# ZhenghaoFei/visual_odom

Hardware: AMD Instinct MI355X
Metric: stereo frames/sec on KITTI-00 1241x376 @ ~2000 features (higher is better)
Workload: dtype u8/int32 LK (f32 2x2 solve), f64 pose solve

## Files before the change

visual_odom_amd/csrc/lk.hip:

```cpp
#include "vo_kernels.h"
#include "vo_lkmath.h"

#include <float.h>
#include <type_traits>

namespace vo {

constexpr int LK_WIN = 21;
constexpr int LK_JT_W = 48, LK_JT_H = 40;
constexpr int LK_W_BITS = 14;
template <int W>
struct LkWin {
    static_assert(W % 2 == 1 && W >= 5 && W <= LK_WIN, "odd windows of 5 .. 21: the pyramid's borders are laid out for 21");
    static constexpr int SEGS = (W + 6) / 7, LANES = W * SEGS, COLS = 7 * SEGS + 1, ROWS = W + 1, LAST = W - 7 * (SEGS - 1);
    static constexpr int OFF_X = ((LK_JT_W - COLS) / 2) & ~3, OFF_Y = (LK_JT_H - ROWS) / 2;
    static_assert(LANES <= 64 && LK_JT_W >= COLS + OFF_X + 3 && LK_JT_H >= ROWS + OFF_Y, "the lane map and the tile hold the window");
};
constexpr uint32_t lk_seg_mask(int valid, int m)
{
    return (2 * m < valid ? 0x0000ffffu : 0u) | (2 * m + 1 < valid ? 0xffff0000u : 0u);
}

__device__ __forceinline__ void lk_weights(float a, float b, uint32_t &wt, uint32_t &wb)
{
    const float s = (float)(1 << LK_W_BITS), magic = 12582912.f;
    const float a1 = (1.f - a) * s, a0 = a * s, b1 = 1.f - b;
    const uint32_t r00 = (uint32_t)__float_as_int(a1 * b1 + magic);
    const uint32_t r01 = (uint32_t)__float_as_int(a0 * b1 + magic);
    const uint32_t r10 = (uint32_t)__float_as_int(a1 * b + magic);
    const uint32_t iw11 = ((1u << LK_W_BITS) + 3u * 0x4B400000u) - (r00 + r01 + r10);
    wt = perm_b32(r01, r00, VO_SEL_LO16);
    wb = perm_b32(iw11, r10, VO_SEL_LO16);
}

struct LkOrigin {
    int x, y;
};
template <int W = LK_WIN>
__device__ __forceinline__ bool lk_tile_misses(bool have_tile, int jx0, int jy0, int inx, int iny)
{
    return !have_tile || inx < jx0 || inx + LkWin<W>::COLS > jx0 + LK_JT_W || iny < jy0 || iny + LkWin<W>::ROWS > jy0 + LK_JT_H;
}
template <int W = LK_WIN>
__device__ __forceinline__ LkOrigin lk_tile_refill(uint8_t *tile, const VO_GLOBAL uint8_t *__restrict__ Jimg, int jstride, int jx_max, int jy_max,
                                               int inx, int iny, int c0, int step)
{
    int jx0 = (inx - LkWin<W>::OFF_X) & ~3;
    int jy0 = iny - LkWin<W>::OFF_Y;
    jx0 = jx0 < -VO_BX ? -VO_BX : jx0 > jx_max ? jx_max : jx0;
    jy0 = jy0 < -VO_BY ? -VO_BY : jy0 > jy_max ? jy_max : jy0;
    const VO_GLOBAL uint8_t *tb = Jimg + (ptrdiff_t)jy0 * jstride + jx0;
    for (int c = c0; c < LK_JT_H * (LK_JT_W / 16); c += step) {
        const int row = c / (LK_JT_W / 16), col = c - row * (LK_JT_W / 16);
        const U32x4A4 v = *(const VO_GLOBAL U32x4A4 *)(tb + (uint32_t)(row * jstride + 16 * col));
        *reinterpret_cast<uint4 *>(&tile[row * LK_JT_W + 16 * col]) = make_uint4(v.a, v.b, v.c, v.d);
    }
    return LkOrigin{jx0, jy0};
}
template <int W = LK_WIN>
__device__ __forceinline__ LkOrigin lk_tile_cover(uint8_t *tile, const VO_GLOBAL uint8_t *__restrict__ Jimg, int jstride, int jx_max, int jy_max,
                                              int inx, int iny, int lane, bool have_tile, int jx0, int jy0)
{
    if (!lk_tile_misses<W>(have_tile, jx0, jy0, inx, iny))
        return LkOrigin{jx0, jy0};
    __syncthreads();
    const LkOrigin o = lk_tile_refill<W>(tile, Jimg, jstride, jx_max, jy_max, inx, iny, lane, 64);
    __syncthreads();
    return o;
}
__device__ __forceinline__ void lk_cell_rows(const uint8_t *tile, int off, uint32_t Jt[7], uint32_t Jb[7])
{
    const U32x2A1 t = *reinterpret_cast<const U32x2A1 *>(&tile[off]);
    const U32x2A1 u = *reinterpret_cast<const U32x2A1 *>(&tile[off + LK_JT_W]);
    lift7(t.a, t.b, Jt);
    lift7(u.a, u.b, Jb);
}

#ifndef VO_LK_ATTRS
#define VO_LK_ATTRS __launch_bounds__(64, 7)
#endif
constexpr int VO_LK_USE_INITIAL_FLOW = 4, VO_LK_GET_MIN_EIGENVALS = 8;
template <bool SPLIT, bool ERR, int WIN = LK_WIN, bool FLAGS = false>
__device__ __forceinline__ void lk_circular_body(const PyrImage *__restrict__ imgs, const Quad *__restrict__ quads,
                                                 const float2 *__restrict__ pts_in, const int *__restrict__ n_pts, int cap,
                                                 int n_frames, int fpg , int ppp ,
                                                 float2 *__restrict__ trk,
                                                 uint8_t *__restrict__ status,
                                                 const LkParams prm, int hop_begin, int hop_end, float *__restrict__ err = nullptr,
                                                 int flags = 0)
{
    __shared__ __attribute__((aligned(16))) uint8_t s_jt[LK_JT_H * LK_JT_W];

    const int bid = blockIdx.x;
    const int xcd = bid & 7, slot = bid >> 3;
    const int grp = slot / ppp, fi = slot - grp * ppp;
    const int frame = grp * fpg + (xcd & (fpg - 1));
    const int f = (xcd / fpg) * ppp + fi;
    if (frame >= n_frames || f >= n_pts[frame])
        return;
    const int lane = threadIdx.x;
    using LW = LkWin<WIN>;
    const bool live = lane < LW::LANES;
    const int lr = live ? lane : LW::LANES - 1;
    const int r = lr / LW::SEGS, c0 = 7 * (lr - LW::SEGS * r);
    const int lane_off = r * LK_JT_W + c0;

    const Quad q = quads[frame];
    const float halfWin = (WIN - 1) * 0.5f;
    const float FLT_SCALE = 1.f / (1 << 20);
    const float eps_lo = (float)(prm.epsilon * 0.999999), eps_hi = (float)(prm.epsilon * 1.000001);
    const float min_eig_n = prm.min_eig * (1.001f * (float)(2 * WIN * WIN));

    const float2 p = pts_in[(size_t)frame * cap + f];
    float prevPtX = unif(p.x), prevPtY = unif(p.y);
    if (SPLIT && hop_begin > 0) {
        const size_t o = ((size_t)frame * 4 + (hop_begin - 1)) * cap + f;
        const float2 q0 = trk[o];
        const bool dead0 = status[o] == 0 || q0.x < 0.f || q0.y < 0.f || (hop_begin == 1 && (p.x < 0.f || p.y < 0.f));
        if (dead0 && !prm.full_chain)
            return;
        prevPtX = unif(q0.x);
        prevPtY = unif(q0.y);
    }

    for (int hop = SPLIT ? hop_begin : 0; hop < (ERR ? 1 : SPLIT ? hop_end : 4); hop++) {
        const int pi = hop == 0 ? q.l0 : hop == 1 ? q.r0 : hop == 2 ? q.r1 : q.l1;
        const int ni = hop == 0 ? q.r0 : hop == 1 ? q.r1 : hop == 2 ? q.l1 : q.l0;
        const PyrImage &I = imgs[pi];
        const PyrImage &J = imgs[ni];
        float outX = 0.f, outY = 0.f;
        int st = 1;
        float errv = 0.f;

        for (int level = prm.max_level; level >= 0; level--) {
            const float scale = __int_as_float((127 - level) << 23);
            float prevX = prevPtX * scale, prevY = prevPtY * scale;
            float nextX, nextY;
            if (level == prm.max_level) {
                nextX = prevX;
                nextY = prevY;
                if constexpr (FLAGS) {
                    if (flags & VO_LK_USE_INITIAL_FLOW) {
                        const float2 g = trk[(size_t)frame * cap + f];
                        nextX = unif(g.x) * scale;
                        nextY = unif(g.y) * scale;
                    }
                }
            } else {
                nextX = outX * 2.f;
                nextY = outY * 2.f;
            }
            outX = nextX;
            outY = nextY;

            const int iw = I.w[level], ih = I.h[level], istride = I.stride[level];
            const int jw = J.w[level], jh = J.h[level], jstride = J.stride[level];
            const VO_GLOBAL uint8_t *__restrict__ Iimg = (const VO_GLOBAL uint8_t *)I.lvl[level];
            const VO_GLOBAL uint32_t *__restrict__ Ider = (const VO_GLOBAL uint32_t *)I.der[level];
            const VO_GLOBAL uint8_t *__restrict__ Jimg = (const VO_GLOBAL uint8_t *)J.lvl[level];

            prevX -= halfWin;
            prevY -= halfWin;
            const float fpx = floorf(prevX), fpy = floorf(prevY);
            const int ipx = uni(vo_f2i(fpx)), ipy = uni(vo_f2i(fpy));
            if (VO_BALLOT(__builtin_isunordered(fpx, fpy)) != 0ull || ipx < -WIN || ipx >= iw || ipy < -WIN || ipy >= ih) {
                if (level == 0)
                    st = 0;
                continue;
            }
            uint32_t wt, wb;
            lk_weights(prevX - fpx, prevY - fpy, wt, wb);

            uint32_t Ixp[4], Iyp[4];
            uint32_t Ipe[ERR ? 4 : 1];
            int a11 = 0, a12 = 0, a22 = 0, c1 = 0, c2 = 0;
            {
                const ptrdiff_t org = (ptrdiff_t)VO_BY * istride + VO_BX;
                const VO_GLOBAL uint8_t *Ib = Iimg - org;
                const VO_GLOBAL uint8_t *Db = (const VO_GLOBAL uint8_t *)(Ider - org);
                const uint32_t o = (uint32_t)((ipy + r + VO_BY) * istride + ipx + c0 + VO_BX);
                const uint32_t od = live ? 4u * o : 0u, drow = 4u * (uint32_t)istride;
                const U32x2A1 t = *(const VO_GLOBAL U32x2A1 *)(Ib + o);
                const U32x2A1 u = *(const VO_GLOBAL U32x2A1 *)(Ib + (o + (uint32_t)istride));
                const U32x4A4 dt0 = *(const VO_GLOBAL U32x4A4 *)(Db + od);
                const U32x4A4 dt1 = *(const VO_GLOBAL U32x4A4 *)(Db + (od + 16u));
                const U32x4A4 db0 = *(const VO_GLOBAL U32x4A4 *)(Db + (od + drow));
                const U32x4A4 db1 = *(const VO_GLOBAL U32x4A4 *)(Db + (od + drow + 16u));
                const uint32_t dt[8] = {dt0.a, dt0.b, dt0.c, dt0.d, dt1.a, dt1.b, dt1.c, dt1.d};
                const uint32_t db[8] = {db0.a, db0.b, db0.c, db0.d, db1.a, db1.b, db1.c, db1.d};
                uint32_t Ip[4];
                bilinear7_u8(t.a, t.b, u.a, u.b, wt, wb, Ip);
                bilinear7_deriv(dt, db, wt, wb, Ixp, Iyp);
                if constexpr (LW::LAST < 7) {
                    const bool part = LW::SEGS == 1 || c0 == 7 * (LW::SEGS - 1);
#pragma unroll
                    for (int m = 0; m < 4; m++) {
                        const uint32_t keep = part ? lk_seg_mask(LW::LAST, m) : 0xffffffffu;
                        Ixp[m] &= keep;
                        Iyp[m] &= keep;
                    }
                }
                a11 = sdot2_first(Ixp[0], Ixp[0], 0);
                a12 = sdot2_first(Ixp[0], Iyp[0], 0);
                a22 = sdot2_first(Iyp[0], Iyp[0], 0);
                c1 = sdot2_first(Ip[0], Ixp[0], 0);
                c2 = sdot2_first(Ip[0], Iyp[0], 0);
#pragma unroll
                for (int m = 1; m < 4; m++) {
                    a11 = sdot2(Ixp[m], Ixp[m], a11);
                    a12 = sdot2(Ixp[m], Iyp[m], a12);
                    a22 = sdot2(Iyp[m], Iyp[m], a22);
                    c1 = sdot2(Ip[m], Ixp[m], c1);
                    c2 = sdot2(Ip[m], Iyp[m], c2);
                }
                if constexpr (ERR) {
#pragma unroll
                    for (int m = 0; m < 4; m++)
                        Ipe[m] = Ip[m];
                }
            }
            float A11, A12, A22;
            wave_sum3_exact_f32(a11, a12, a22, A11, A12, A22);
            A11 *= FLT_SCALE;
            A12 *= FLT_SCALE;
            A22 *= FLT_SCALE;

            float D = A11 * A22 - A12 * A12;
            const float t = A22 + A11;
            const float s2 = (A11 - A22) * (A11 - A22) + 4.f * A12 * A12;
            const float u = t - (min_eig_n + t * 3.814697265625e-6f);
            bool eig_ok = u > 0.f && s2 < u * u * 0.9999f;
            if (__builtin_expect(!eig_ok, 0)) {
#ifndef VO_HOST_EMUL
                asm volatile("" ::: "memory");
#endif
                const float minEig = (t - sqrtf(s2)) / (float)(2 * WIN * WIN);
                eig_ok = !(minEig < prm.min_eig);
            }
            if constexpr (FLAGS) {
                if ((flags & VO_LK_GET_MIN_EIGENVALS) && level == 0)
                    errv = (t - sqrtf(s2)) / (float)(2 * WIN * WIN);
            }
            if (!eig_ok || D < FLT_EPSILON) {
                if (level == 0)
                    st = 0;
                continue;
            }
            D = 1.f / D;
            const float A11s = A11 * FLT_SCALE, A12s = A12 * FLT_SCALE, A22s = A22 * FLT_SCALE;
            const int nc1 = -c1, nc2 = -c2;

            nextX -= halfWin;
            nextY -= halfWin;
            float prevDX = 0.f, prevDY = 0.f;
            int jx0 = 0, jy0 = 0;
            bool have_tile = false;
            static_assert(LK_JT_W % 16 == 0 && VO_BX % 4 == 0, "16-byte tile chunks at 4-byte aligned origins");
            static_assert(VO_BY >= WIN && LK_JT_W >= LW::COLS + LW::OFF_X + 3 && LK_JT_H >= LW::ROWS + LW::OFF_Y,
                          "a tile clamped to the row end / the last border row still covers what the window of every corner the "
                          "reference admits reads (up to w - 1, h - 1: the borders are at least a window wide)");
            static_assert(VO_BY >= LW::COLS - 1, "right border (at least VO_BY columns) >= the columns a row reads beyond corner w - 1");
            const int jx_max = jstride - VO_BX - LK_JT_W, jy_max = jh + VO_BY - LK_JT_H;

            int j = 0;
            float fnx = floorf(nextX), fny = floorf(nextY);
            bool run = prm.max_count > 0;
            while (run) {
                const int inx = uni(vo_f2i(fnx)), iny = uni(vo_f2i(fny));
                if (VO_BALLOT(__builtin_isunordered(fnx, fny)) != 0ull || inx < -WIN || inx >= jw || iny < -WIN || iny >= jh) {
                    if (level == 0)
                        st = 0;
                    break;
                }
                {
                    const LkOrigin o = lk_tile_cover<WIN>(s_jt, Jimg, jstride, jx_max, jy_max, inx, iny, lane, have_tile, jx0, jy0);
                    jx0 = o.x;
                    jy0 = o.y;
                    have_tile = true;
                }
                uint32_t Jt[7], Jb[7];
                lk_cell_rows(s_jt, (iny - jy0) * LK_JT_W + (inx - jx0) + lane_off, Jt, Jb);
                for (;;) {
                    lk_weights(nextX - fnx, nextY - fny, wt, wb);
                    int b1, b2;
                    {
                        uint32_t Jp[4];
                        blend7(Jt, Jb, wt, wb, Jp);
                        b1 = sdot2_first(Jp[0], Ixp[0], nc1);
                        b2 = sdot2_first(Jp[0], Iyp[0], nc2);
#pragma unroll
                        for (int m = 1; m < 4; m++) {
                            b1 = sdot2(Jp[m], Ixp[m], b1);
                            b2 = sdot2(Jp[m], Iyp[m], b2);
                        }
                    }
                    float fb1, fb2;
                    wave_sum2_exact_f32(b1, b2, fb1, fb2);
                    const float dx = (A12s * fb2 - A22s * fb1) * D;
                    const float dy = (A12s * fb1 - A11s * fb2) * D;
                    nextX += dx;
                    nextY += dy;
                    outX = nextX + halfWin;
                    outY = nextY + halfWin;
                    const float n2 = fmaf(dy, dy, dx * dx);
                    if (__builtin_expect(!(n2 > eps_hi), 0)) {
#ifndef VO_HOST_EMUL
                        asm volatile("" ::: "memory");
#endif
                        if (n2 < eps_lo || (double)dx * dx + (double)dy * dy <= prm.epsilon) {
                            run = false;
                            break;
                        }
                    }
                    if (j > 0 && fabsf(dx + prevDX) <= 0.01f && fabsf(dy + prevDY) <= 0.01f) {
#ifndef VO_HOST_EMUL
                        asm volatile("" ::: "memory");
#endif
                        outX -= dx * 0.5f;
                        outY -= dy * 0.5f;
                        run = false;
                        break;
                    }
                    prevDX = dx;
                    prevDY = dy;
                    if (++j >= prm.max_count) {
                        run = false;
                        break;
                    }
                    const uint32_t ua = (uint32_t)__float_as_int(nextX - fnx), ub = (uint32_t)__float_as_int(nextY - fny);
                    if (VO_BALLOT((ua > ub ? ua : ub) >= 0x3f800000u) != 0ull) {
                        fnx = floorf(nextX);
                        fny = floorf(nextY);
                        break;
                    }
                }
            }

            if (st && level == 0 && (!FLAGS || !(flags & VO_LK_GET_MIN_EIGENVALS))) {
                const int fx = vo_f2i(floorf(outX - halfWin)), fy = vo_f2i(floorf(outY - halfWin));
                if (fx < -WIN || fx >= jw || fy < -WIN || fy >= jh)
                    st = 0;
                if constexpr (ERR) {
                    if (st && err != nullptr) {
                        const float ex = outX - halfWin, ey = outY - halfWin;
                        const float fex = floorf(ex), fey = floorf(ey);
                        const int inx = uni(fx), iny = uni(fy);
                        const LkOrigin o = lk_tile_cover<WIN>(s_jt, Jimg, jstride, jx_max, jy_max, inx, iny, lane, have_tile, jx0, jy0);
                        jx0 = o.x;
                        jy0 = o.y;
                        uint32_t Jt[7], Jb[7], Jp[4];
                        lk_cell_rows(s_jt, (iny - jy0) * LK_JT_W + (inx - jx0) + lane_off, Jt, Jb);
                        lk_weights(ex - fex, ey - fey, wt, wb);
                        blend7(Jt, Jb, wt, wb, Jp);
                        uint32_t e = 0;
#pragma unroll
                        for (int m = 0; m < 4; m++) {
                            if constexpr (LW::LAST < 7) {
                                const bool part = LW::SEGS == 1 || c0 == 7 * (LW::SEGS - 1);
                                e = udot2(pk_absdiff_i16(Jp[m], Ipe[m]) & (part ? lk_seg_mask(LW::LAST, m) : 0xffffffffu), 0x00010001u, e);
                            } else
                                e = udot2(pk_absdiff_i16(Jp[m], Ipe[m]), 0x00010001u, e);
                        }
                        errv = wave_sum_exact_f32(live ? (int)e : 0) / (float)(32 * WIN * WIN);
                    }
                }
            }
        }

        if constexpr (ERR) {
            if (lane == 0) {
                trk[(size_t)frame * cap + f] = make_float2(outX, outY);
                status[(size_t)frame * cap + f] = (uint8_t)st;
                if (err != nullptr) {
                    if constexpr (FLAGS)
                        err[(size_t)frame * cap + f] = ((flags & VO_LK_GET_MIN_EIGENVALS) || st) ? errv : 0.f;
                    else
                        err[(size_t)frame * cap + f] = st ? errv : 0.f;
                }
            }
            return;
        }
        if (lane == 0) {
            trk[((size_t)frame * 4 + hop) * cap + f] = make_float2(outX, outY);
            status[((size_t)frame * 4 + hop) * cap + f] = (uint8_t)st;
        }
        const bool dead = st == 0 || outX < 0.f || outY < 0.f || (hop == 0 && (p.x < 0.f || p.y < 0.f));
        if (dead && !prm.full_chain && hop < 3) {
            if (lane == 0)
                for (int k = hop + 1; k < 4; k++) {
                    trk[((size_t)frame * 4 + k) * cap + f] = make_float2(-1.f, -1.f);
                    status[((size_t)frame * 4 + k) * cap + f] = 0;
                }
            return;
        }
        prevPtX = unif(outX);
        prevPtY = unif(outY);
    }
}

__global__ VO_LK_ATTRS void lk_circular_kernel(const PyrImage *__restrict__ imgs,
                                                          const Quad *__restrict__ quads,
                                                          const float2 *__restrict__ pts_in,
                                                          const int *__restrict__ n_pts, int cap,
                                                          int n_frames, int fpg ,
                                                          int ppp ,
                                                          float2 *__restrict__ trk,
                                                          uint8_t *__restrict__ status,
                                                          LkParams prm)
{
    lk_circular_body<false, false>(imgs, quads, pts_in, n_pts, cap, n_frames, fpg, ppp, trk, status, prm, 0, 4);
}

__global__ VO_LK_ATTRS void lk_hops_kernel(const PyrImage *__restrict__ imgs, const Quad *__restrict__ quads,
                                           const float2 *__restrict__ pts_in, const int *__restrict__ n_pts, int cap,
                                           int n_frames, int fpg, int ppp, float2 *__restrict__ trk,
                                           uint8_t *__restrict__ status, LkParams prm, int hop_begin, int hop_end)
{
    lk_circular_body<true, false>(imgs, quads, pts_in, n_pts, cap, n_frames, fpg, ppp, trk, status, prm, hop_begin, hop_end);
}

#ifndef VO_LK_FLOW_ATTRS
#define VO_LK_FLOW_ATTRS __launch_bounds__(64, 6)
#endif
__global__ VO_LK_FLOW_ATTRS void lk_flow_kernel(const PyrImage *__restrict__ imgs, const Quad *__restrict__ pairs,
                                                const float2 *__restrict__ pts_in, const int *__restrict__ n_pts, int cap,
                                                int n_frames, int fpg, int ppp, float2 *__restrict__ next,
                                                uint8_t *__restrict__ status,
                                                float *__restrict__ err , LkParams prm)
{
    lk_circular_body<false, true>(imgs, pairs, pts_in, n_pts, cap, n_frames, fpg, ppp, next, status, prm, 0, 1, err);
}

template <int W>
__global__ VO_LK_FLOW_ATTRS void lk_flow_win_kernel(const PyrImage *__restrict__ imgs, const Quad *__restrict__ pairs,
                                                    const float2 *__restrict__ pts_in, const int *__restrict__ n_pts, int cap,
                                                    int n_frames, int fpg, int ppp, float2 *__restrict__ next,
                                                    uint8_t *__restrict__ status,
                                                    float *__restrict__ err , LkParams prm)
{
    static_assert(W < LK_WIN, "21 is lk_flow_kernel");
    lk_circular_body<false, true, W>(imgs, pairs, pts_in, n_pts, cap, n_frames, fpg, ppp, next, status, prm, 0, 1, err);
}

template <int W>
__global__ VO_LK_FLOW_ATTRS void lk_flow_flags_kernel(const PyrImage *__restrict__ imgs, const Quad *__restrict__ pairs,
                                                      const float2 *__restrict__ pts_in, const int *__restrict__ n_pts, int cap,
                                                      int n_frames, int fpg, int ppp, float2 *__restrict__ next,
                                                      uint8_t *__restrict__ status,
                                                      float *__restrict__ err , LkParams prm, int flags)
{
    lk_circular_body<false, true, W, true>(imgs, pairs, pts_in, n_pts, cap, n_frames, fpg, ppp, next, status, prm, 0, 1, err, flags);
}

struct LkGrid {
    int fpg, ppp, blocks;
};
inline LkGrid lk_grid(int n_frames, int n_items)
{
    const int fpg = n_frames >= 8 ? 8 : n_frames >= 4 ? 4 : n_frames >= 2 ? 2 : 1;
    const int parts = 8 / fpg, ppp = (n_items + parts - 1) / parts;
    const int groups = (n_frames + fpg - 1) / fpg;
    return {fpg, ppp, 8 * groups * ppp};
}

template <int... W, typename F>
inline bool lk_visit_window(int win, F &&f)
{
    return ((win == W && (f(std::integral_constant<int, W>{}), true)) || ...);
}
template <typename F>
inline bool lk_for_window(int win, F &&f)
{
    return lk_visit_window<5, 7, 9, 11, 13, 15, 17, 19, LK_WIN>(win, f);
}

template <int W, typename R>
inline void lk_flow_route(int flags, R &&run)
{
    if (flags != 0)
        run(lk_flow_flags_kernel<W>, flags);
    else if constexpr (W == LK_WIN)
        run(lk_flow_kernel);
    else
        run(lk_flow_win_kernel<W>);
}

#ifndef VO_HOST_EMUL
void launch_lk_flow(int win, int flags, const PyrImage *d_imgs, const Quad *d_pairs, const float2 *d_pts, const int *d_npts, int cap,
                    int max_pts, int n_frames, float2 *d_next, uint8_t *d_status, float *d_err, const LkParams &prm, hipStream_t stream)
{
    if (max_pts <= 0 || n_frames <= 0 || (flags & ~(VO_LK_USE_INITIAL_FLOW | VO_LK_GET_MIN_EIGENVALS)))
        return;
    const LkGrid g = lk_grid(n_frames, max_pts);
    lk_for_window(win, [&](auto w) {
        lk_flow_route<decltype(w)::value>(flags, [&](auto kernel, auto... tail) {
            hipLaunchKernelGGL(kernel, dim3((unsigned)g.blocks), dim3(64), 0, stream, d_imgs, d_pairs, d_pts, d_npts, cap, n_frames, g.fpg,
                               g.ppp, d_next, d_status, d_err, prm, tail...);
        });
    });
}

void launch_lk_circular(const PyrImage *d_imgs, const Quad *d_quads, const float2 *d_pts, const int *d_npts,
                        int cap, int max_pts, int n_frames, float2 *d_trk, uint8_t *d_status,
                        const LkParams &prm, hipStream_t stream)
{
    if (max_pts <= 0 || n_frames <= 0)
        return;
    const LkGrid g = lk_grid(n_frames, max_pts);
    hipLaunchKernelGGL(lk_circular_kernel, dim3((unsigned)g.blocks), dim3(64), 0, stream, d_imgs, d_quads, d_pts, d_npts, cap,
                       n_frames, g.fpg, g.ppp, d_trk, d_status, prm);
}

void launch_lk_hops(const PyrImage *d_imgs, const Quad *d_quads, const float2 *d_pts, const int *d_npts, int cap, int max_pts,
                    int n_frames, float2 *d_trk, uint8_t *d_status, const LkParams &prm, int hop_begin, int hop_end,
                    hipStream_t stream)
{
    if (max_pts <= 0 || n_frames <= 0 || hop_begin < 0 || hop_end > 4 || hop_begin >= hop_end)
        return;
    const LkGrid g = lk_grid(n_frames, max_pts);
    hipLaunchKernelGGL(lk_hops_kernel, dim3((unsigned)g.blocks), dim3(64), 0, stream, d_imgs, d_quads, d_pts, d_npts, cap, n_frames,
                       g.fpg, g.ppp, d_trk, d_status, prm, hop_begin, hop_end);
}

#endif

}

#ifdef VO_HOST_EMUL
#include "dev/lk_dev.hip"
#endif
```

visual_odom_amd/csrc/vo_lkmath.h:

```cpp
#pragma once

#include "vo_isa.h"

namespace vo {

#define VO_SEL_PIX(k) (0x0cu | ((uint32_t)(k) << 8) | (0x0cu << 16) | ((uint32_t)((k) + 1) << 24))
constexpr uint32_t VO_SEL_LO16 = 0x05040100u;
constexpr uint32_t VO_SEL_HI16 = 0x07060302u;

VO_HD uint32_t pack_w(int w_lo, int w_hi)
{
#if defined(__HIP_DEVICE_COMPILE__)
    return __builtin_bit_cast(uint32_t, __builtin_amdgcn_cvt_pk_i16(w_lo, w_hi));
#else
    return (uint32_t)(w_lo & 0xffff) | ((uint32_t)w_hi << 16);
#endif
}

VO_HD void bilinear7_u8(uint32_t t_lo, uint32_t t_hi, uint32_t b_lo, uint32_t b_hi, uint32_t wt, uint32_t wb,
                        uint32_t out[4])
{
    uint32_t acc[8];
    if (!(wb & 0x80000000u)) {
#define VO_PIX_STEP(k)                                                                               \
    acc[k] = udot2(perm_b32(b_hi, b_lo, VO_SEL_PIX(k)), wb,                                          \
                   udot2(perm_b32(t_hi, t_lo, VO_SEL_PIX(k)), wt, 1u << 16));
        VO_PIX_STEP(0) VO_PIX_STEP(1) VO_PIX_STEP(2) VO_PIX_STEP(3) VO_PIX_STEP(4) VO_PIX_STEP(5) VO_PIX_STEP(6)
#undef VO_PIX_STEP
    } else {
        const uint32_t wb0 = wb & 0xffffu, kneg = (uint32_t)(-(int32_t)((int16_t)(wb >> 16)));
#define VO_PIX_STEP(k)                                                                               \
    {                                                                                                \
        const uint32_t pb = perm_b32(b_hi, b_lo, VO_SEL_PIX(k));                                     \
        acc[k] = udot2(pb, wb0, udot2(perm_b32(t_hi, t_lo, VO_SEL_PIX(k)), wt, 1u << 16)) -          \
                 kneg * (pb >> 16);                                                                  \
    }
        VO_PIX_STEP(0) VO_PIX_STEP(1) VO_PIX_STEP(2) VO_PIX_STEP(3) VO_PIX_STEP(4) VO_PIX_STEP(5) VO_PIX_STEP(6)
#undef VO_PIX_STEP
    }
    acc[7] = 0;
#pragma unroll
    for (int m = 0; m < 4; m++)
        out[m] = pk_lshr1_u16(perm_b32(acc[2 * m + 1], acc[2 * m], VO_SEL_HI16));
}

VO_HD void lift7(uint32_t lo, uint32_t hi, uint32_t pair[7])
{
#define VO_LIFT(k) pair[k] = perm_b32(hi, lo, VO_SEL_PIX(k));
    VO_LIFT(0) VO_LIFT(1) VO_LIFT(2) VO_LIFT(3) VO_LIFT(4) VO_LIFT(5) VO_LIFT(6)
#undef VO_LIFT
}

VO_HD void blend7(const uint32_t pt[7], const uint32_t pb[7], uint32_t wt, uint32_t wb, uint32_t out[4])
{
    uint32_t acc[8];
    if (!(wb & 0x80000000u)) {
#pragma unroll
        for (int k = 0; k < 7; k++)
            acc[k] = udot2(pb[k], wb, udot2(pt[k], wt, 1u << 16));
    } else {
        const uint32_t wb0 = wb & 0xffffu, kneg = (uint32_t)(-(int32_t)((int16_t)(wb >> 16)));
#pragma unroll
        for (int k = 0; k < 7; k++)
            acc[k] = udot2(pb[k], wb0, udot2(pt[k], wt, 1u << 16)) - kneg * (pb[k] >> 16);
    }
    acc[7] = 0;
#pragma unroll
    for (int m = 0; m < 4; m++)
        out[m] = pk_lshr1_u16(perm_b32(acc[2 * m + 1], acc[2 * m], VO_SEL_HI16));
}

VO_HD void bilinear7_deriv(const uint32_t dt[8], const uint32_t db[8], uint32_t wt, uint32_t wb, uint32_t ix[4],
                           uint32_t iy[4])
{
    int32_t ax[8], ay[8];
#pragma unroll
    for (int k = 0; k < 7; k++) {
        ax[k] = sdot2(perm_b32(db[k + 1], db[k], VO_SEL_LO16), wb,
                      sdot2_first(perm_b32(dt[k + 1], dt[k], VO_SEL_LO16), wt, 1 << 15));
        ay[k] = sdot2(perm_b32(db[k + 1], db[k], VO_SEL_HI16), wb,
                      sdot2_first(perm_b32(dt[k + 1], dt[k], VO_SEL_HI16), wt, 1 << 15));
    }
    ax[7] = ay[7] = 0;
#pragma unroll
    for (int m = 0; m < 4; m++) {
        ix[m] = perm_b32((uint32_t)ax[2 * m + 1], (uint32_t)ax[2 * m], VO_SEL_HI16);
        iy[m] = perm_b32((uint32_t)ay[2 * m + 1], (uint32_t)ay[2 * m], VO_SEL_HI16);
    }
}

VO_HD uint32_t scharr4_packed(int p00, int p01, int p02, int p10, int p12, int p20, int p21, int p22)
{
    int ix = ((p02 + p22) * 3 + p12 * 10) - ((p00 + p20) * 3 + p10 * 10);
    int iy = ((p22 - p02) + (p20 - p00)) * 3 + (p21 - p01) * 10;
    return ((uint32_t)(ix * 4) & 0xffffu) | ((uint32_t)(iy * 4) << 16);
}

}
```

Baseline: 22480.

## Pack bilinear samples by columns and refill the LK tile with a one-wave loop

Switches the packed bilinear interpolation from row pairs (top/bottom) to column pairs (left/right). Eight lifted columns are shared between adjacent pixels, so the J cell needs 8 permutes instead of 14 and fewer registers, and the derivative path gets the same layout. It also replaces the strided tile-refill loop with a fixed two-chunks-per-lane load using a multiply-shift row index. The cost is a different weight packing and more intricate address arithmetic, which could introduce rounding or indexing mismatches.

```diff
diff --git a/visual_odom_amd/csrc/lk.hip b/visual_odom_amd/csrc/lk.hip
--- a/visual_odom_amd/csrc/lk.hip
+++ b/visual_odom_amd/csrc/lk.hip
@@ -21,7 +21,8 @@
     return (2 * m < valid ? 0x0000ffffu : 0u) | (2 * m + 1 < valid ? 0xffff0000u : 0u);
 }
 
-__device__ __forceinline__ void lk_weights(float a, float b, uint32_t &wt, uint32_t &wb)
+template <bool COLS>
+__device__ __forceinline__ void lk_weights_packed(float a, float b, uint32_t &w0, uint32_t &w1)
 {
     const float s = (float)(1 << LK_W_BITS), magic = 12582912.f;
     const float a1 = (1.f - a) * s, a0 = a * s, b1 = 1.f - b;
@@ -29,8 +30,16 @@
     const uint32_t r01 = (uint32_t)__float_as_int(a0 * b1 + magic);
     const uint32_t r10 = (uint32_t)__float_as_int(a1 * b + magic);
     const uint32_t iw11 = ((1u << LK_W_BITS) + 3u * 0x4B400000u) - (r00 + r01 + r10);
-    wt = perm_b32(r01, r00, VO_SEL_LO16);
-    wb = perm_b32(iw11, r10, VO_SEL_LO16);
+    w0 = perm_b32(COLS ? r10 : r01, r00, VO_SEL_LO16);
+    w1 = perm_b32(iw11, COLS ? r01 : r10, VO_SEL_LO16);
+}
+__device__ __forceinline__ void lk_weights(float a, float b, uint32_t &wt, uint32_t &wb)
+{
+    lk_weights_packed<false>(a, b, wt, wb);
+}
+__device__ __forceinline__ void lk_weights_cols(float a, float b, uint32_t &wl, uint32_t &wr)
+{
+    lk_weights_packed<true>(a, b, wl, wr);
 }
 
 struct LkOrigin {
@@ -42,20 +51,52 @@
     return !have_tile || inx < jx0 || inx + LkWin<W>::COLS > jx0 + LK_JT_W || iny < jy0 || iny + LkWin<W>::ROWS > jy0 + LK_JT_H;
 }
 template <int W = LK_WIN>
-__device__ __forceinline__ LkOrigin lk_tile_refill(uint8_t *tile, const VO_GLOBAL uint8_t *__restrict__ Jimg, int jstride, int jx_max, int jy_max,
-                                               int inx, int iny, int c0, int step)
+__device__ __forceinline__ LkOrigin lk_tile_origin(int jx_max, int jy_max, int inx, int iny)
 {
     int jx0 = (inx - LkWin<W>::OFF_X) & ~3;
     int jy0 = iny - LkWin<W>::OFF_Y;
     jx0 = jx0 < -VO_BX ? -VO_BX : jx0 > jx_max ? jx_max : jx0;
     jy0 = jy0 < -VO_BY ? -VO_BY : jy0 > jy_max ? jy_max : jy0;
+    return LkOrigin{jx0, jy0};
+}
+template <int W = LK_WIN>
+__device__ __forceinline__ LkOrigin lk_tile_refill(uint8_t *tile, const VO_GLOBAL uint8_t *__restrict__ Jimg, int jstride, int jx_max, int jy_max,
+                                               int inx, int iny, int c0, int step)
+{
+    const LkOrigin org = lk_tile_origin<W>(jx_max, jy_max, inx, iny);
+    const int jx0 = org.x, jy0 = org.y;
     const VO_GLOBAL uint8_t *tb = Jimg + (ptrdiff_t)jy0 * jstride + jx0;
     for (int c = c0; c < LK_JT_H * (LK_JT_W / 16); c += step) {
         const int row = c / (LK_JT_W / 16), col = c - row * (LK_JT_W / 16);
         const U32x4A4 v = *(const VO_GLOBAL U32x4A4 *)(tb + (uint32_t)(row * jstride + 16 * col));
         *reinterpret_cast<uint4 *>(&tile[row * LK_JT_W + 16 * col]) = make_uint4(v.a, v.b, v.c, v.d);
     }
-    return LkOrigin{jx0, jy0};
+    return org;
+}
+template <int W = LK_WIN>
+__device__ __forceinline__ LkOrigin lk_tile_refill_wave(uint8_t *tile, const VO_GLOBAL uint8_t *__restrict__ Jimg, int jstride, int jx_max,
+                                                    int jy_max, int inx, int iny, int lane)
+{
+    constexpr int CPR = LK_JT_W / 16, CHUNKS = LK_JT_H * CPR;
+    static_assert(CPR == 3 && CHUNKS > 64 && CHUNKS <= 128, "two chunks per lane at most; 64 chunks = 21 rows + 1 chunk");
+    const LkOrigin org = lk_tile_origin<W>(jx_max, jy_max, inx, iny);
+    const VO_GLOBAL uint8_t *tb = Jimg + (ptrdiff_t)org.y * jstride + org.x;
+#ifndef VO_HOST_EMUL
+    asm volatile("" : "+v"(lane));
+#endif
+    const int row = (lane * 43) >> 7, col = lane - CPR * row;
+    const uint32_t g0 = (uint32_t)(row * jstride + 16 * col);
+    const int next_col = 21 * jstride + 16, next_row = 22 * jstride - 16 * (CPR - 1);
+    const uint32_t g1 = g0 + (uint32_t)(col == CPR - 1 ? next_row : next_col);
+    const bool second = lane < CHUNKS - 64;
+    const U32x4A4 v0 = *(const VO_GLOBAL U32x4A4 *)(tb + g0);
+    U32x4A4 v1 = v0;
+    if (second)
+        v1 = *(const VO_GLOBAL U32x4A4 *)(tb + g1);
+    *reinterpret_cast<uint4 *>(&tile[16 * lane]) = make_uint4(v0.a, v0.b, v0.c, v0.d);
+    if (second)
+        *reinterpret_cast<uint4 *>(&tile[16 * lane + 1024]) = make_uint4(v1.a, v1.b, v1.c, v1.d);
+    return org;
 }
 template <int W = LK_WIN>
 __device__ __forceinline__ LkOrigin lk_tile_cover(uint8_t *tile, const VO_GLOBAL uint8_t *__restrict__ Jimg, int jstride, int jx_max, int jy_max,
@@ -64,7 +105,7 @@
     if (!lk_tile_misses<W>(have_tile, jx0, jy0, inx, iny))
         return LkOrigin{jx0, jy0};
     __syncthreads();
-    const LkOrigin o = lk_tile_refill<W>(tile, Jimg, jstride, jx_max, jy_max, inx, iny, lane, 64);
+    const LkOrigin o = lk_tile_refill_wave<W>(tile, Jimg, jstride, jx_max, jy_max, inx, iny, lane);
     __syncthreads();
     return o;
 }
@@ -74,6 +115,12 @@
     const U32x2A1 u = *reinterpret_cast<const U32x2A1 *>(&tile[off + LK_JT_W]);
     lift7(t.a, t.b, Jt);
     lift7(u.a, u.b, Jb);
+}
+__device__ __forceinline__ void lk_cell_cols(const uint8_t *tile, int off, uint32_t Jc[8])
+{
+    const U32x2A1 t = *reinterpret_cast<const U32x2A1 *>(&tile[off]);
+    const U32x2A1 u = *reinterpret_cast<const U32x2A1 *>(&tile[off + LK_JT_W]);
+    lift8_cols(t.a, t.b, u.a, u.b, Jc);
 }
 
 #ifndef VO_LK_ATTRS
@@ -168,8 +215,8 @@
                     st = 0;
                 continue;
             }
-            uint32_t wt, wb;
-            lk_weights(prevX - fpx, prevY - fpy, wt, wb);
+            uint32_t wl, wr;
+            lk_weights_cols(prevX - fpx, prevY - fpy, wl, wr);
 
             uint32_t Ixp[4], Iyp[4];
             uint32_t Ipe[ERR ? 4 : 1];
@@ -189,8 +236,8 @@
                 const uint32_t dt[8] = {dt0.a, dt0.b, dt0.c, dt0.d, dt1.a, dt1.b, dt1.c, dt1.d};
                 const uint32_t db[8] = {db0.a, db0.b, db0.c, db0.d, db1.a, db1.b, db1.c, db1.d};
                 uint32_t Ip[4];
-                bilinear7_u8(t.a, t.b, u.a, u.b, wt, wb, Ip);
-                bilinear7_deriv(dt, db, wt, wb, Ixp, Iyp);
+                bilinear7_u8_cols(t.a, t.b, u.a, u.b, wl, wr, Ip);
+                bilinear7_deriv_cols(dt, db, wl, wr, Ixp, Iyp);
                 if constexpr (LW::LAST < 7) {
                     const bool part = LW::SEGS == 1 || c0 == 7 * (LW::SEGS - 1);
 #pragma unroll
@@ -278,14 +325,14 @@
                     jy0 = o.y;
                     have_tile = true;
                 }
-                uint32_t Jt[7], Jb[7];
-                lk_cell_rows(s_jt, (iny - jy0) * LK_JT_W + (inx - jx0) + lane_off, Jt, Jb);
+                uint32_t Jc[8];
+                lk_cell_cols(s_jt, (iny - jy0) * LK_JT_W + (inx - jx0) + lane_off, Jc);
                 for (;;) {
-                    lk_weights(nextX - fnx, nextY - fny, wt, wb);
+                    lk_weights_cols(nextX - fnx, nextY - fny, wl, wr);
                     int b1, b2;
                     {
                         uint32_t Jp[4];
-                        blend7(Jt, Jb, wt, wb, Jp);
+                        blend7_cols(Jc, wl, wr, Jp);
                         b1 = sdot2_first(Jp[0], Ixp[0], nc1);
                         b2 = sdot2_first(Jp[0], Iyp[0], nc2);
 #pragma unroll
@@ -348,10 +395,10 @@
                         const LkOrigin o = lk_tile_cover<WIN>(s_jt, Jimg, jstride, jx_max, jy_max, inx, iny, lane, have_tile, jx0, jy0);
                         jx0 = o.x;
                         jy0 = o.y;
-                        uint32_t Jt[7], Jb[7], Jp[4];
-                        lk_cell_rows(s_jt, (iny - jy0) * LK_JT_W + (inx - jx0) + lane_off, Jt, Jb);
-                        lk_weights(ex - fex, ey - fey, wt, wb);
-                        blend7(Jt, Jb, wt, wb, Jp);
+                        uint32_t Jc[8], Jp[4];
+                        lk_cell_cols(s_jt, (iny - jy0) * LK_JT_W + (inx - jx0) + lane_off, Jc);
+                        lk_weights_cols(ex - fex, ey - fey, wl, wr);
+                        blend7_cols(Jc, wl, wr, Jp);
                         uint32_t e = 0;
 #pragma unroll
                         for (int m = 0; m < 4; m++) {
diff --git a/visual_odom_amd/csrc/vo_lkmath.h b/visual_odom_amd/csrc/vo_lkmath.h
--- a/visual_odom_amd/csrc/vo_lkmath.h
+++ b/visual_odom_amd/csrc/vo_lkmath.h
@@ -70,6 +70,46 @@
         out[m] = pk_lshr1_u16(perm_b32(acc[2 * m + 1], acc[2 * m], VO_SEL_HI16));
 }
 
+#define VO_SEL_COL(k) (0x0cu | ((uint32_t)(k) << 8) | (0x0cu << 16) | ((uint32_t)((k) + 4) << 24))
+VO_HD void lift8_cols(uint32_t t_lo, uint32_t t_hi, uint32_t b_lo, uint32_t b_hi, uint32_t col[8])
+{
+#define VO_LIFT(k) col[k] = perm_b32(b_lo, t_lo, VO_SEL_COL(k)), col[(k) + 4] = perm_b32(b_hi, t_hi, VO_SEL_COL(k));
+    VO_LIFT(0) VO_LIFT(1) VO_LIFT(2) VO_LIFT(3)
+#undef VO_LIFT
+}
+
+VO_HD void blend7_cols(const uint32_t col[8], uint32_t wl, uint32_t wr, uint32_t out[4])
+{
+    uint32_t acc[8];
+    if (!(wr & 0x80000000u)) {
+#pragma unroll
+        for (int k = 0; k < 7; k++)
+            acc[k] = udot2(col[k + 1], wr, udot2(col[k], wl, 1u << 16));
+    } else {
+        const uint32_t wr0 = wr & 0xffffu, kneg = (uint32_t)(-(int32_t)((int16_t)(wr >> 16)));
+#pragma unroll
+        for (int k = 0; k < 7; k++) {
+            uint32_t c = col[k + 1];
+#if defined(__HIP_DEVICE_COMPILE__)
+            asm volatile("" : "+v"(c));
+#endif
+            acc[k] = udot2(c, wr0, udot2(col[k], wl, 1u << 16)) - kneg * (c >> 16);
+        }
+    }
+    acc[7] = 0;
+#pragma unroll
+    for (int m = 0; m < 4; m++)
+        out[m] = pk_lshr1_u16(perm_b32(acc[2 * m + 1], acc[2 * m], VO_SEL_HI16));
+}
+
+VO_HD void bilinear7_u8_cols(uint32_t t_lo, uint32_t t_hi, uint32_t b_lo, uint32_t b_hi, uint32_t wl, uint32_t wr,
+                             uint32_t out[4])
+{
+    uint32_t col[8];
+    lift8_cols(t_lo, t_hi, b_lo, b_hi, col);
+    blend7_cols(col, wl, wr, out);
+}
+
 VO_HD void bilinear7_deriv(const uint32_t dt[8], const uint32_t db[8], uint32_t wt, uint32_t wb, uint32_t ix[4],
                            uint32_t iy[4])
 {
@@ -89,6 +129,29 @@
     }
 }
 
+VO_HD void bilinear7_deriv_cols(const uint32_t dt[8], const uint32_t db[8], uint32_t wl, uint32_t wr, uint32_t ix[4],
+                                uint32_t iy[4])
+{
+    uint32_t cx[8], cy[8];
+    int32_t ax[8], ay[8];
+#pragma unroll
+    for (int k = 0; k < 8; k++) {
+        cx[k] = perm_b32(db[k], dt[k], VO_SEL_LO16);
+        cy[k] = perm_b32(db[k], dt[k], VO_SEL_HI16);
+    }
+#pragma unroll
+    for (int k = 0; k < 7; k++) {
+        ax[k] = sdot2(cx[k + 1], wr, sdot2_first(cx[k], wl, 1 << 15));
+        ay[k] = sdot2(cy[k + 1], wr, sdot2_first(cy[k], wl, 1 << 15));
+    }
+    ax[7] = ay[7] = 0;
+#pragma unroll
+    for (int m = 0; m < 4; m++) {
+        ix[m] = perm_b32((uint32_t)ax[2 * m + 1], (uint32_t)ax[2 * m], VO_SEL_HI16);
+        iy[m] = perm_b32((uint32_t)ay[2 * m + 1], (uint32_t)ay[2 * m], VO_SEL_HI16);
+    }
+}
+
 VO_HD uint32_t scharr4_packed(int p00, int p01, int p02, int p10, int p12, int p20, int p21, int p22)
 {
     int ix = ((p02 + p22) * 3 + p12 * 10) - ((p00 + p20) * 3 + p10 * 10);
```

Measured after the change: 23490, median of 6. 4.5% higher.
